# laboshinl/loam_velodyne

Hardware: AMD Instinct MI355X
Metric: sweeps/sec (64-ring, 1M-pt map): feature extraction + odometry + scan-to-map registration (higher is better)
Workload: dtype f32

## Files before the change

### loam_velodyne_amd/csrc/odometry.hip

```cpp
#include "odometry.hpp"
#include "odom_schedule.hpp"
#include "pinned_copy.hpp"
#include <chrono>
#include <cstring>
#include <type_traits>

namespace loamx {

constexpr int OD_THREADS = 256;
constexpr int OD_TR_STRIDE = OD_THREADS + 2;
constexpr int OD_PART_STRIDE = 2 * (2 * 16 * LX_NSUM) + 16;
[[maybe_unused]] constexpr int OD_PART_TS = 2 * (2 * 16 * LX_NSUM);

__device__ inline void sincos_f(float a, float& s, float& c) { sincosf(a, &s, &c); }

__device__ inline void transform_to_start(const float* T, float scan_period, const float4 pi, float& x, float& y, float& z) {
  const float s = (1.f / scan_period) * (pi.w - (float)(int)pi.w);
  x = pi.x - s * T[3];
  y = pi.y - s * T[4];
  z = pi.z - s * T[5];
  float sx, cx, sy, cy, sz, cz;
  sincos_f(-s * T[0], sx, cx);
  sincos_f(-s * T[1], sy, cy);
  sincos_f(-s * T[2], sz, cz);
// ... 107 lines not shown
      v = cell_start[((uint32_t)z * g.ny + y) * g.nx + xx];
    }
  }
  uint32_t acc = 0;
#pragma unroll
  for (int r = 0; r < 9; r++) {
    const uint32_t b = (uint32_t)__shfl((int)v, 2 * r, 64), e = (uint32_t)__shfl((int)v, 2 * r + 1, 64);
    B.O[r] = b - acc;
    acc += e > b ? e - b : 0u;
    B.E[r] = acc;
  }
  B.total = acc;
}
#ifndef OD_BLK_CACHE
#define OD_BLK_CACHE 2
#endif
struct Block27First { float4 p[OD_BLK_CACHE > 0 ? OD_BLK_CACHE : 1]; };
template <bool LOAD_FIRST, class F>
__device__ inline void block27_scan(const Block27& B, const float4* __restrict__ sorted, int lane, Block27First& first, F&& visit) {
  for (uint32_t c0 = (uint32_t)lane; c0 < B.total; c0 += 4 * 64) {
    const bool first_trip = c0 == (uint32_t)lane;
    uint32_t pos[4];
    float4 p[4];
#pragma unroll
    for (int u = 0; u < 4; u++) {
      const uint32_t cc = c0 + 64u * u;
      uint32_t o = B.O[8];
#pragma unroll
      for (int k = 7; k >= 0; k--) o = cc < B.E[k] ? B.O[k] : o;
      pos[u] = cc < B.total ? cc + o : B.O[0];
    }
    if (LOAD_FIRST || !first_trip) {
#pragma unroll
      for (int u = 0; u < 4; u++) p[u] = sorted[pos[u]];
      if (LOAD_FIRST && first_trip) {
#pragma unroll
        for (int u = 0; u < OD_BLK_CACHE; u++) first.p[u] = p[u];
      }
    } else {
#pragma unroll
      for (int u = OD_BLK_CACHE; u < 4; u++) p[u] = sorted[pos[u]];
#pragma unroll
      for (int u = 0; u < OD_BLK_CACHE; u++) p[u] = first.p[u];
    }
#pragma unroll
    for (int u = 0; u < 4; u++) visit(p[u], (c0 + 64u * u) < B.total);
  }
}
__device__ inline int nn1_block(const GridDesc& g, const Block27& B, const float4* __restrict__ sorted, const uint32_t* __restrict__ cell_start,
                                float qx, float qy, float qz, int lane, uint32_t& w_out, Block27First& first) {
  float lbest = 25.0f;
  uint32_t lw = 0xffffffffu;
  block27_scan<true>(B, sorted, lane, first, [&](const float4& p, bool valid) {
    const float dx = qx - p.x, dy2 = qy - p.y, dz2 = qz - p.z;
    const float d2 = dx * dx + dy2 * dy2 + dz2 * dz2;
    const uint32_t w = __float_as_uint(p.w);
    if (valid && (d2 < lbest || (d2 == lbest && lw != 0xffffffffu && (w & OD_IDX_MASK) < (lw & OD_IDX_MASK)))) { lbest = d2; lw = w; }
  });
  float d = lbest;
  int j = lw == 0xffffffffu ? -1 : (int)(lw & OD_IDX_MASK), o_ = lw == 0xffffffffu ? 0x7fffffff : (int)(lw & OD_IDX_MASK);
  int ring = (int)(lw >> 24);
  {
#pragma unroll
    for (int off = 32; off > 0; off >>= 1) {
      const float od = __shfl_xor(d, off, 64);
      const int oj = __shfl_xor(j, off, 64), oo = __shfl_xor(o_, off, 64), orr = __shfl_xor(ring, off, 64);
      if (od < d || (od == d && oo < o_)) { d = od; j = oj; o_ = oo; ring = orr; }
    }
  }
  const float h = 1.0f / g.inv_h;
  if (j >= 0 && d < 25.0f && d <= h * h) { w_out = ((uint32_t)ring << 24) | (uint32_t)j; return j; }
  const int id = nn1_shells(g, sorted, cell_start, qx, qy, qz, lane, 2, (j >= 0 && d < 25.0f) ? d : 25.0f, (j >= 0 && d < 25.0f) ? j : -1);
  w_out = id == j ? (((uint32_t)ring << 24) | (uint32_t)j) : (0xff000000u | (uint32_t)(id < 0 ? 0 : id));
  return id;
}

constexpr int OD_RF_N = 320;
#ifdef LOAMX_PROF_CORR
__device__ unsigned long long g_corr_ts[3][16];
#define OC_TS(k) do { if (blockIdx.y == 0 && lane == 0 && ts_slot >= 0) g_corr_ts[ts_slot][k] = wall_clock64(); } while (0)
#else
#define OC_TS(k) do { } while (0)
#endif
__global__ __launch_bounds__(256) OD_CORR_ATTR void k_odom_corr_grid(OdomProblem* __restrict__ probs, OdomParams P, uint32_t* __restrict__ patch_dst, uint4 patch) {
  if (patch_dst && blockIdx.x == 0 && blockIdx.y == 0 && threadIdx.x == 0) { patch_dst[0] = patch.x; patch_dst[1] = patch.y; patch_dst[2] = patch.z; }
  OdomProblem& pb = probs[blockIdx.y];
  if (pb.done) return;
  const int lane = threadIdx.x & 63, wid = threadIdx.x >> 6;
  const int nSharp = (int)pb.n_sharp, nFlat = (int)pb.n_flat;
  int f;
  {
    const int x = (int)(blockIdx.x % 8), j = (int)(blockIdx.x / 8);
    const int sS = (int)((long long)x * nSharp / 8), nS = (int)((long long)(x + 1) * nSharp / 8) - sS;
    const int sF = (int)((long long)x * nFlat / 8), nF = (int)((long long)(x + 1) * nFlat / 8) - sF;
    const int fl = 4 * j + wid;
    if (fl >= nS + nF) return;
    f = fl < nS ? sS + fl : nSharp + sF + (fl - nS);
  }
#ifdef LOAMX_PROF_CORR
  const int ts_slot = f == nSharp / 2 ? 0 : f == nSharp + nFlat / 2 ? 1 : f == nSharp + nFlat - 1 ? 2 : -1;
#endif
  OC_TS(0);
  float T[6];
#pragma unroll
  for (int k = 0; k < 6; k++) T[k] = pb.transform[k];
  const bool corner = f < nSharp;
  const float4 pi = corner ? pb.sharp[f] : pb.flat[f - nSharp];
  const uint32_t* __restrict__ tbl = corner ? pb.rf_corner : pb.rf_surf;
  const int e0 = max((int)pi.w - 8, 0);
  uint32_t tv = 0u, unordered_epoch = 0u;
  if (tbl) {
    if (e0 + lane < OD_RF_N - 1) tv = tbl[e0 + lane];
    unordered_epoch = tbl[OD_RF_N - 1];
  }
  float x, y, z;
  transform_to_start(T, P.scan_period, pi, x, y, z);
  const GridDescB gd = corner ? *pb.lc_desc : *pb.ls_desc;
  const float4* __restrict__ sorted = pb.sorted;
  const uint32_t* __restrict__ cell_start = pb.cell_table + gd.cell_base;
  OC_TS(1);
  Block27 B;
  block27_build(gd.g, cell_start, x, y, z, lane, B);
  OC_TS(2);
  uint32_t wbest = 0u;
  Block27First first;
  const int closest = nn1_block(gd.g, B, sorted, cell_start, x, y, z, lane, wbest, first);
  OC_TS(3);
  if (closest < 0) {
    if (lane == 0) { pb.ind[5 * f] = -1; pb.ind[5 * f + 1] = -1; pb.ind[5 * f + 2] = -1; }
    return;
  }
  const float4* last = corner ? pb.last_corner : pb.last_surf;
  const int nLast = corner ? (int)pb.n_last_corner : (int)pb.n_last_surf;
  const int nCur = corner ? nSharp : nFlat;
  const int bound = nCur < nLast ? nCur : nLast;
  const int cscan = (wbest >> 24) != 255u ? (int)(wbest >> 24) : (int)last[closest].w;
  float d2 = 25.f, d3 = 25.f;
  int j2 = -1, j3 = -1, o2 = 0x7fffffff, o3 = 0x7fffffff;
  auto better = [](float d, int order, float dbest, int obest) { return d < dbest || (d == dbest && obest != 0x7fffffff && order < obest); };

  bool via_block = false;
  if (tbl && unordered_epoch != pb.rf_epoch && cscan < 255 && B.total > 0u) {
    const unsigned long long valid = __ballot(e0 + lane < OD_RF_N - 1 && (tv >> 24) == pb.rf_epoch);
    auto first_from = [&](int ring) -> int {
      const int k = ring - e0;
      if (k >= 64) return nLast;
      const unsigned long long m = k <= 0 ? valid : (valid >> k) << k;
      if (!m) return nLast;
      const int w = (int)((uint32_t)__shfl((int)tv, __builtin_ctzll(m), 64) & OD_IDX_MASK);
      return w < nLast ? w : nLast;
    };
    if (cscan - 2 >= e0 || e0 == 0) {
      const int wlo = min(first_from(cscan - 2), closest);
      const int whi = closest + 1 < bound ? max(min(bound, first_from(cscan + 3)), closest + 1) : closest + 1;
      const unsigned walk = (unsigned)(closest - wlo) + (unsigned)(whi - (closest + 1));
      via_block = walk > B.total + 128u;
    }
  }
  OC_TS(4);
  if (via_block) {
    block27_scan<false>(B, sorted, lane, first, [&](const float4& p, bool ok) {
      const uint32_t w = __float_as_uint(p.w);
      const int j = (int)(w & OD_IDX_MASK), ring = (int)(w >> 24);
      const float d = sqd(p, x, y, z);
      if (ok && j > closest && j < bound && ring <= cscan + 2) {
        const int order = j - (closest + 1);
        if (corner) {
          if (ring > cscan && better(d, order, d2, o2)) { d2 = d; j2 = j; o2 = order; }
        } else {
          if (ring <= cscan) { if (better(d, order, d2, o2)) { d2 = d; j2 = j; o2 = order; } }
          else { if (better(d, order, d3, o3)) { d3 = d; j3 = j; o3 = order; } }
        }
      } else if (ok && j < closest && ring >= cscan - 2) {
        const int order = 0x40000000 + (closest - 1 - j);
        if (corner) {
          if (ring < cscan && better(d, order, d2, o2)) { d2 = d; j2 = j; o2 = order; }
        } else {
          if (ring >= cscan) { if (better(d, order, d2, o2)) { d2 = d; j2 = j; o2 = order; } }
          else { if (better(d, order, d3, o3)) { d3 = d; j3 = j; o3 = order; } }
        }
      }
    });
    wave_argmin(d2, j2, o2);
    if (!corner) wave_argmin(d3, j3, o3);
    const float h = 1.0f / gd.g.inv_h, h2 = h * h;
    via_block = d2 < h2 && (corner || d3 < h2);
    if (!via_block) { d2 = d3 = 25.f; j2 = j3 = -1; o2 = o3 = 0x7fffffff; }
  }
  OC_TS(5);
  if (!via_block) {
    int baseF = closest + 1, baseB = closest - 1;
    bool stopF = baseF >= bound, stopB = baseB < 0;
    while (!stopF || !stopB) {
      float4 qf[4], qb[4];
      if (!stopF) {
#pragma unroll
        for (int u = 0; u < 4; u++) {
          const int j = baseF + 64 * u + lane;
          qf[u] = j < bound ? last[j] : make_float4(0.f, 0.f, 0.f, 0.f);
        }
      }
      if (!stopB) {
#pragma unroll
        for (int u = 0; u < 4; u++) {
          const int j = baseB - 64 * u - lane;
          qb[u] = j >= 0 ? last[j] : make_float4(0.f, 0.f, 0.f, 0.f);
        }
      }
      if (!stopF) {
        bool stop = false;
#pragma unroll
        for (int u = 0; u < 4; u++) {
          if (stop) continue;
          const int j = baseF + 64 * u + lane;
          const bool in = j < bound;
          const int ring = (int)qf[u].w;
          const bool brk = in && ((double)ring > (double)cscan + 2.5);
          const unsigned long long mb = __ballot(brk);
          const int fb = mb ? __builtin_ctzll(mb) : 64;
          if (in && lane < fb) {
            const float d = sqd(qf[u], x, y, z);
            const int order = j - (closest + 1);
            if (corner) {
              if (ring > cscan && better(d, order, d2, o2)) { d2 = d; j2 = j; o2 = order; }
            } else {
              if (ring <= cscan) { if (better(d, order, d2, o2)) { d2 = d; j2 = j; o2 = order; } }
              else { if (better(d, order, d3, o3)) { d3 = d; j3 = j; o3 = order; } }
            }
          }
          if (mb) stop = true;
        }
        baseF += 256;
        stopF = stop || baseF >= bound;
      }
      if (!stopB) {
        bool stop = false;
#pragma unroll
        for (int u = 0; u < 4; u++) {
          if (stop) continue;
          const int j = baseB - 64 * u - lane;
          const bool in = j >= 0;
          const int ring = (int)qb[u].w;
          const bool brk = in && ((double)ring < (double)cscan - 2.5);
          const unsigned long long mb = __ballot(brk);
          const int fb = mb ? __builtin_ctzll(mb) : 64;
          if (in && lane < fb) {
            const float d = sqd(qb[u], x, y, z);
            const int order = 0x40000000 + (closest - 1 - j);
            if (corner) {
              if (ring < cscan && better(d, order, d2, o2)) { d2 = d; j2 = j; o2 = order; }
            } else {
              if (ring >= cscan) { if (better(d, order, d2, o2)) { d2 = d; j2 = j; o2 = order; } }
              else { if (better(d, order, d3, o3)) { d3 = d; j3 = j; o3 = order; } }
            }
          }
          if (mb) stop = true;
        }
        baseB -= 256;
        stopB = stop || baseB < 0;
      }
    }
    wave_argmin(d2, j2, o2);
    if (!corner) wave_argmin(d3, j3, o3);
  }
  OC_TS(6);
  if (lane == 0) {
    pb.ind[5 * f] = closest;
    pb.ind[5 * f + 1] = j2;
    pb.ind[5 * f + 2] = corner ? -1 : j3;
  }
#ifdef LOAMX_PROF_CORR
  if (blockIdx.y == 0 && lane == 0 && ts_slot >= 0) {
    g_corr_ts[ts_slot][7] = wall_clock64();
    g_corr_ts[ts_slot][8] = (unsigned long long)B.total; g_corr_ts[ts_slot][9] = (unsigned long long)via_block;
    g_corr_ts[ts_slot][10] = (unsigned long long)closest; g_corr_ts[ts_slot][11] = (unsigned long long)cscan;
  }
#endif
}

#ifdef LOAMX_PROF_LM
#define LM_TS(k) do { if (blockIdx.x == 0 && blockIdx.y == 0 && tid == 0 && iter == it_begin + 1) pb.part[OD_PART_TS + (k)] = (double)wall_clock64(); } while (0)
#else
#define LM_TS(k) do { } while (0)
#endif
#ifndef OD_LM_WAVES
#define OD_LM_WAVES 3
#endif
#ifndef OD_LM_WAVES_MIN
#define OD_LM_WAVES_MIN 3
#endif
#define OD_LM_ATTR __attribute__((amdgpu_waves_per_eu(OD_LM_WAVES_MIN, OD_LM_WAVES)))
#pragma clang diagnostic push
#pragma clang diagnostic ignored "-Wpass-failed"
template <int OD_FPT>
__global__ __launch_bounds__(OD_THREADS) OD_LM_ATTR void k_odom_lm(OdomProblem* __restrict__ probs, OdomParams P, int iter0, int n_iters) {
  OdomProblem& pb = probs[blockIdx.y];
  if (pb.done) return;
  const unsigned NB = gridDim.x;
  const int tid = threadIdx.x;
  const int nSharp = (int)pb.n_sharp, nFlat = (int)pb.n_flat, nFeat = nSharp + nFlat;
  __shared__ float T[6];
  __shared__ float trig[6];
  __shared__ double red[8][LX_NSUM];
  using TrT = typename std::conditional<OD_FPT == 1, float, double>::type;
  __shared__ TrT tr[LX_NSUM * OD_TR_STRIDE];
  __shared__ int sh_done, sh_degen, sh_abort;
  __shared__ float matP[36];
  __shared__ float ws[216];
  __shared__ double parts[16 * LX_NSUM];
  __shared__ float AtA[36], AtB[6];
  if (tid < 6) {
    T[tid] = pb.transform[tid];
    const double ang = (double)pb.transform[tid >> 1];
    trig[tid] = (float)((tid & 1) ? cos(ang) : sin(ang));
  }
  const unsigned xtag = pb.xchg_epoch << 8;
  if (tid == 0) { sh_done = 0; sh_abort = 0; sh_degen = pb.stats.degenerate; }
  if (tid < 36) matP[tid] = pb.matP[tid];
  __syncthreads();

  float4 fpo[OD_FPT], ft1[OD_FPT], ft2[OD_FPT], ft3[OD_FPT];
  bool fvalid[OD_FPT], fcorner[OD_FPT];
#pragma unroll
  for (int u = 0; u < OD_FPT; u++) {
    const int f = (u * (int)NB + (int)blockIdx.x) * OD_THREADS + tid;
    fvalid[u] = false;
    fcorner[u] = f < nSharp;
    fpo[u] = ft1[u] = ft2[u] = ft3[u] = make_float4(0.f, 0.f, 0.f, 0.f);
    if (f < nFeat) {
      const int i1 = pb.ind[5 * f], i2 = pb.ind[5 * f + 1], i3 = pb.ind[5 * f + 2];
      if (fcorner[u] ? (i2 >= 0) : (i2 >= 0 && i3 >= 0)) {
        fvalid[u] = true;
        fpo[u] = fcorner[u] ? pb.sharp[f] : pb.flat[f - nSharp];
        const float4* last = fcorner[u] ? pb.last_corner : pb.last_surf;
        ft1[u] = last[i1];
        ft2[u] = last[i2];
        if (!fcorner[u]) ft3[u] = last[i3];
      }
    }
  }

  const int it_begin = iter0, it_end = iter0 + n_iters;
  for (int iter = it_begin; iter < it_end; iter++) {
    LM_TS(0);
    LM_TS(1);
    double v[OD_FPT == 1 ? 1 : LX_NSUM];
    float a1[6] = {0.f, 0.f, 0.f, 0.f, 0.f, 0.f}, bb1 = 0.f;
    bool sel1 = false;
#pragma unroll
    for (int k = 0; k < (OD_FPT == 1 ? 1 : LX_NSUM); k++) v[k] = 0.0;
#pragma unroll
    for (int u = 0; u < OD_FPT; u++) {
      if (!fvalid[u]) continue;
      const bool corner = fcorner[u];
      const float4 po = fpo[u];
      float cx = 0.f, cy = 0.f, cz = 0.f, ci = 0.f;
      bool sel = false;
      {
        float x0, y0, z0;
        transform_to_start(T, P.scan_period, po, x0, y0, z0);
        if (corner) {
// ... 361 lines not shown
void OdometryBatch::lt_resolve_() {
  for (auto& c : lt_) {
    if (!c.pending || !c.pairs) continue;
    if (hipEventQuery(c.ev[3 * (c.pairs - 1) + 2]) != hipSuccess) { (void)hipGetLastError(); continue; }
    for (int k = 0; k < c.pairs; k++) {
      float a = 0.f, b = 0.f;
      if (hipEventElapsedTime(&a, c.ev[3 * k], c.ev[3 * k + 1]) != hipSuccess || hipEventElapsedTime(&b, c.ev[3 * k + 1], c.ev[3 * k + 2]) != hipSuccess) { (void)hipGetLastError(); continue; }
      if (c.iters[k] > 0) {
        lt_tot_.corr_ms += a; lt_tot_.corr_launches++; lt_tot_.corr_features += c.feats[k];
        lt_tot_.lm_ms += b; lt_tot_.lm_launches++; lt_tot_.lm_iterations += (uint64_t)c.iters[k]; lt_tot_.lm_bytes += c.bytes[k];
      } else {
        lt_tot_.corr_noop_ms += a; lt_tot_.corr_noop_launches++;
        lt_tot_.lm_noop_ms += b; lt_tot_.lm_noop_launches++;
      }
    }
    c.pending = false;
  }
}
OdometryBatch::LaunchTotals OdometryBatch::launch_totals() {
  std::lock_guard<std::mutex> lk(lt_mu_);
  lt_resolve_();
  return lt_tot_;
}

void odom_set_imu(OdomStream& S, const float* t);
ToEndParams odom_to_end_params(const OdomStream& S, float scan_period, bool enabled);
void odom_integrate_pose(OdomStream& S);

void OdometryBatch::update_imu(uint32_t s, const float* t) { odom_set_imu(*streams_[s], t); }

ToEndParams OdometryBatch::to_end_params(uint32_t s, bool enabled) const { return odom_to_end_params(*streams_[s], params.scan_period, enabled); }

void OdometryBatch::to_end_device(uint32_t s, float4* pts, uint32_t n) {
  if (!n) return;
  hipLaunchKernelGGL(k_transform_to_end, dim3((n + 255) / 256), dim3(256), 0, st_, pts, n, to_end_params(s, true));
}

void odom_integrate_pose(OdomStream& S) {
  HAngle rx, ry, rz;
  accumulate_rotation(S.transform_sum.rot_x, S.transform_sum.rot_y, S.transform_sum.rot_z, -S.transform.rot_x,
                      HAngle((float)(-S.transform.rot_y.r * 1.05)), -S.transform.rot_z, rx, ry, rz);
  HVec3 v{S.transform.pos.x - S.imu_shift.x, S.transform.pos.y - S.imu_shift.y, (float)(S.transform.pos.z * 1.05 - S.imu_shift.z)};
  h_rot_zxy(v, rz, rx, ry);
  HVec3 trans{S.transform_sum.pos.x - v.x, S.transform_sum.pos.y - v.y, S.transform_sum.pos.z - v.z};
  plugin_imu_rotation(rx, ry, rz, S.imu_pitch_start, S.imu_yaw_start, S.imu_roll_start, S.imu_pitch_end, S.imu_yaw_end,
                      S.imu_roll_end, rx, ry, rz);
  S.transform_sum.rot_x = rx; S.transform_sum.rot_y = ry; S.transform_sum.rot_z = rz;
  S.transform_sum.pos = trans;
}
void odom_set_imu(OdomStream& S, const float* t) {
  S.imu_pitch_start = HAngle(t[0]); S.imu_yaw_start = HAngle(t[1]); S.imu_roll_start = HAngle(t[2]);
  S.imu_pitch_end = HAngle(t[3]); S.imu_yaw_end = HAngle(t[4]); S.imu_roll_end = HAngle(t[5]);
  S.imu_shift = {t[6], t[7], t[8]};
  S.imu_velo = {t[9], t[10], t[11]};
}
ToEndParams odom_to_end_params(const OdomStream& S, float scan_period, bool enabled) {
  ToEndParams P;
  S.transform.get(P.T);
  const HAngle* ta[3] = {&S.transform.rot_x, &S.transform.rot_y, &S.transform.rot_z};
  const HAngle* sa[3] = {&S.imu_pitch_start, &S.imu_yaw_start, &S.imu_roll_start};
  const HAngle* ea[3] = {&S.imu_pitch_end, &S.imu_yaw_end, &S.imu_roll_end};
  for (int k = 0; k < 3; k++) {
    P.sT[k] = ta[k]->s; P.cT[k] = ta[k]->c;
    P.s_start[k] = sa[k]->s; P.c_start[k] = sa[k]->c;
    P.s_end[k] = ea[k]->s; P.c_end[k] = ea[k]->c;
  }
  P.shift[0] = S.imu_shift.x; P.shift[1] = S.imu_shift.y; P.shift[2] = S.imu_shift.z;
  P.scan_period = scan_period;
  P.enabled = enabled ? 1 : 0;
  return P;
}

struct OdometryBatch::Pass {
  const OdomInput* in;
  int* rc;
  uint32_t ns, K;
  std::vector<OdomInput> in_late;
  bool late_pending = false, patch_pending = false;
  uint32_t n_corner_all = 0, n_all = 0;
  const float4 *src_c = nullptr, *src_s = nullptr;
  std::vector<uint32_t> active;
  uint32_t max_feat = 0, max_sharp = 0, max_flat = 0;
  LtCall* lt = nullptr;
};

void OdometryBatch::process(const OdomInput* in, int* rc, bool defer_tail) {
  TraceRange trace_range("loamx:odometry");
  LX_HIP(hipSetDevice(device_));
  if (up_pending_) {
    LX_HIP(hipEventSynchronize(ev_up_));
    up_pending_ = false;
  }
  Pass p{in, rc, n_streams(), 2 * n_streams()};
  stage_clouds_(p);
  build_problems_(p);
  upload_(p);
  launch_pairs_(p);
  enqueue_tail_(p);
  if (!p.active.empty()) collect_(p);
  integrate_poses_(p);
  if (!defer_tail) {
    LX_HIP(hipStreamSynchronize(st_));
    tail_pending_ = false;
  }
}

void OdometryBatch::stage_clouds_(Pass& p) {
  const uint32_t ns = p.ns;
  p.late_pending = ns == 1 && (bool)late_less_flat;
  if (p.late_pending) {
    p.in_late.assign(p.in, p.in + ns);
    p.in_late[0].less_flat = nullptr; p.in_late[0].n_less_flat = 0;
    p.in = p.in_late.data();
  }
  const OdomInput* in = p.in;
  for (uint32_t s = 0; s < ns; s++) {
    h_cur_off_[s + 1] = h_cur_off_[s] + in[s].n_less_sharp;
    if (s > 0) LX_REQUIRE(in[s].less_sharp == in[s - 1].less_sharp + in[s - 1].n_less_sharp || in[s].n_less_sharp == 0 || in[s - 1].n_less_sharp == 0,
                          "less_sharp clouds of the streams must be contiguous");
  }
  for (uint32_t s = 0; s < ns; s++) h_cur_off_[ns + s + 1] = h_cur_off_[ns + s] + in[s].n_less_flat;
  const uint32_t n_corner_all = p.n_corner_all = h_cur_off_[ns], n_all = p.n_all = h_cur_off_[p.K];
  cur_.reserve((size_t)n_all + (p.late_pending ? late_bound : 0u) + 1);
  bool contig_c = true, contig_s = true;
  for (uint32_t s = 1; s < ns; s++) {
    contig_c = contig_c && in[s].less_sharp == in[s - 1].less_sharp + in[s - 1].n_less_sharp;
    contig_s = contig_s && in[s].less_flat == in[s - 1].less_flat + in[s - 1].n_less_flat;
  }
  if (contig_c && contig_s) { p.src_c = in[0].less_sharp; p.src_s = in[0].less_flat; return; }
  if (contig_c) {
    if (n_corner_all) LX_HIP(hipMemcpyAsync(cur_.p, in[0].less_sharp, sizeof(float4) * n_corner_all, hipMemcpyDeviceToDevice, st_));
  } else {
    for (uint32_t s = 0; s < ns; s++)
      if (in[s].n_less_sharp) LX_HIP(hipMemcpyAsync(cur_.p + h_cur_off_[s], in[s].less_sharp, sizeof(float4) * in[s].n_less_sharp, hipMemcpyDeviceToDevice, st_));
  }
  if (contig_s) {
    if (n_all > n_corner_all) LX_HIP(hipMemcpyAsync(cur_.p + n_corner_all, in[0].less_flat, sizeof(float4) * (n_all - n_corner_all), hipMemcpyDeviceToDevice, st_));
  } else {
    for (uint32_t s = 0; s < ns; s++)
      if (in[s].n_less_flat) LX_HIP(hipMemcpyAsync(cur_.p + h_cur_off_[ns + s], in[s].less_flat, sizeof(float4) * in[s].n_less_flat, hipMemcpyDeviceToDevice, st_));
  }
}

void OdometryBatch::resolve_late_(Pass& p) {
  if (!p.late_pending) return;
  p.late_pending = false;
  const float4* pts = nullptr;
  uint32_t n = 0;
  late_less_flat(pts, n);
  LX_REQUIRE(n <= late_bound, "internal: the late less-flat cloud is larger than its announced bound");
  p.in_late[0].less_flat = pts; p.in_late[0].n_less_flat = n;
  h_cur_off_[p.ns + 1] = h_cur_off_[p.ns] + n;
  p.n_all = h_cur_off_[p.K];
  p.src_s = pts;
  p.patch_pending = true;
}
void OdometryBatch::flush_patch_(Pass& p) {
  if (!p.patch_pending) return;
  p.patch_pending = false;
  h_off_late_.reserve(p.K + 1);
  memcpy(h_off_late_.p, h_cur_off_.data(), sizeof(uint32_t) * (p.K + 1));
  LX_HIP(hipMemcpyAsync(d_cur_off_.p, h_off_late_.p, sizeof(uint32_t) * (p.K + 1), hipMemcpyHostToDevice, st_));
  LX_HIP(hipEventRecord(ev_up_, st_));
}

void OdometryBatch::build_problems_(Pass& p) {
  const uint32_t ns = p.ns;
  xchg_epoch_ = xchg_epoch_ % 0xffffffu + 1u;
  std::vector<uint32_t> ind_off(ns + 1, 0);
  for (uint32_t s = 0; s < ns; s++) ind_off[s + 1] = ind_off[s] + 5 * (p.in[s].n_sharp + p.in[s].n_flat) + 5;
  ind_.reserve(ind_off[ns] + 8);
  for (uint32_t s = 0; s < ns; s++) {
    OdomStream& S = *streams_[s];
    const OdomInput& I = p.in[s];
    if (!S.inited) {
      S.transform_sum.rot_x = HAngle(S.transform_sum.rot_x.r + S.imu_pitch_start.r);
      S.transform_sum.rot_z = HAngle(S.transform_sum.rot_z.r + S.imu_roll_start.r);
      p.rc[s] = LOAMX_SKIPPED;
      continue;
    }
    p.rc[s] = LOAMX_OK;
    S.frame++;
    S.transform.pos.x -= S.imu_velo.x * params.scan_period;
    S.transform.pos.y -= S.imu_velo.y * params.scan_period;
    S.transform.pos.z -= S.imu_velo.z * params.scan_period;
    S.stats = {0, 0, (int)S.frame, 0};
    if (S.n_last_corner > 10 && S.n_last_surf > 100) {
      OdomProblem& pb = h_prob_.p[p.active.size()];
      pb.sharp = I.sharp; pb.n_sharp = I.n_sharp;
      pb.flat = I.flat; pb.n_flat = I.n_flat;
      pb.last_corner = last_.p + h_last_off_[s]; pb.n_last_corner = S.n_last_corner;
      pb.last_surf = last_.p + h_last_off_[ns + s]; pb.n_last_surf = S.n_last_surf;
      pb.sorted = index_.sorted();
      pb.cell_table = index_.cell_table();
      pb.lc_desc = index_.desc(s);
      pb.ls_desc = index_.desc(ns + s);
      pb.ind = ind_.p + ind_off[s];
      S.transform.get(pb.transform);
      pb.stats = {0, 0, 0, 0};
      pb.done = 0;
      pb.ticket = 0;
      pb.xchg_epoch = xchg_epoch_;
      pb.stream_id = (int)s;
      pb.host_mirror = h_mirror_.p + p.active.size();
      pb.te_out = te_.p + s;
      pb.part = part_.p + (size_t)p.active.size() * OD_PART_STRIDE;
      pb.err_word = h_err_.p;
      pb.rf_corner = rf_.p + (size_t)s * OD_RF_N;
      pb.rf_surf = rf_.p + (size_t)(ns + s) * OD_RF_N;
      pb.rf_epoch = rf_epoch_;
      p.max_feat = std::max(p.max_feat, I.n_sharp + I.n_flat);
      p.max_sharp = std::max(p.max_sharp, I.n_sharp);
      p.max_flat = std::max(p.max_flat, I.n_flat);
      p.active.push_back(s);
    }
  }
  if (p.max_feat > 32 * OD_THREADS) throw Error(LOAMX_E_CAPACITY, "more than 8192 sharp+flat features in one sweep");
}

void OdometryBatch::upload_(Pass& p) {
  for (uint32_t s = 0; s < p.ns; s++) h_te_.p[s] = to_end_params(s, p.rc[s] == LOAMX_OK);
  memcpy(h_off_pin_.p, h_cur_off_.data(), sizeof(uint32_t) * (p.K + 1));
  LX_HIP(hipMemcpyAsync(up_dev_.p, up_host_.p, up_bytes_, hipMemcpyHostToDevice, st_));
  index_.prepare(p.K);
  if (!ev_up_) LX_HIP(hipEventCreateWithFlags(&ev_up_, hipEventDisableTiming));
  LX_HIP(hipEventRecord(ev_up_, st_));
  up_pending_ = true;
}

static dim3 odom_corr_grid(uint32_t max_sharp, uint32_t max_flat, uint32_t na) {
  return dim3(8 * (((max_sharp + 7) / 8 + (max_flat + 7) / 8 + 3) / 4), na);
}
OdometryBatch::LmGeometry OdometryBatch::lm_geometry_(uint32_t max_feat) {
#ifdef OD_LM_HALF_WGS
  const uint32_t nb = std::min<uint32_t>(16u, std::max<uint32_t>(1u, (max_feat + 2 * OD_THREADS - 1) / (2 * OD_THREADS)));
#else
  const uint32_t nb = std::min<uint32_t>(16u, (max_feat + OD_THREADS - 1) / OD_THREADS);
#endif
  const bool two = max_feat > nb * OD_THREADS;
  if (!lm_slots_[two]) {
    int per_cu = 0;
    if (two) LX_HIP(hipOccupancyMaxActiveBlocksPerMultiprocessor(&per_cu, k_odom_lm<2>, OD_THREADS, 0));
    else LX_HIP(hipOccupancyMaxActiveBlocksPerMultiprocessor(&per_cu, k_odom_lm<1>, OD_THREADS, 0));
    hipDeviceProp_t prop;
    LX_HIP(hipGetDeviceProperties(&prop, device_));
    lm_slots_[two] = (uint32_t)std::max(per_cu, 1) * (uint32_t)std::max(prop.multiProcessorCount, 1);
  }
  return {nb, two, std::max<uint32_t>(1u, (lm_slots_[two] / 2) / nb)};
}

void OdometryBatch::enqueue_corr_(Pass& p, int k) {
  LtCall* lt = p.lt;
  const int lk = lt && k < LT_MAXP ? k : -1;
  if (lk >= 0) {
    for (int e = 0; e < 3; e++) if (!lt->ev[3 * lk + e]) LX_HIP(hipEventCreate(&lt->ev[3 * lk + e]));
    LX_HIP(hipEventRecord(lt->ev[3 * lk], st_));
  }
  uint32_t* pd = nullptr;
  uint4 pv = make_uint4(0u, 0u, 0u, 0u);
  if (p.patch_pending) { p.patch_pending = false; pd = d_cur_off_.p; pv = make_uint4(h_cur_off_[0], h_cur_off_[1], h_cur_off_[2], 0u); }
  hipLaunchKernelGGL(k_odom_corr_grid, odom_corr_grid(p.max_sharp, p.max_flat, (uint32_t)p.active.size()), dim3(256), 0, st_, prob_.p, params, pd, pv);
  if (lk >= 0) LX_HIP(hipEventRecord(lt->ev[3 * lk + 1], st_));
}
void OdometryBatch::enqueue_lm_(Pass& p, int k) {
  LtCall* lt = p.lt;
  const uint32_t na = (uint32_t)p.active.size();
  const int it0 = 5 * k;
  const int nit = std::min(5, params.max_iterations - it0);
  const int lk = lt && k < LT_MAXP ? k : -1;
  const LmGeometry g = lm_geometry_(p.max_feat);
  for (uint32_t a0 = 0; a0 < na; a0 += g.chunk) {
    const uint32_t nc = std::min(g.chunk, na - a0);
    if (g.two) hipLaunchKernelGGL(k_odom_lm<2>, dim3(g.nb, nc), dim3(OD_THREADS), 0, st_, prob_.p + a0, params, it0, nit);
    else hipLaunchKernelGGL(k_odom_lm<1>, dim3(g.nb, nc), dim3(OD_THREADS), 0, st_, prob_.p + a0, params, it0, nit);
  }
  if (lk >= 0) { LX_HIP(hipEventRecord(lt->ev[3 * lk + 2], st_)); lt->pairs = lk + 1; }
}

struct OdometryBatch::PairOps {
  OdometryBatch& o; Pass& p;
  void corr(int k) { o.enqueue_corr_(p, k); }
  void lm(int k) { o.enqueue_lm_(p, k); }
  void after_first() { o.resolve_late_(p); }
  bool behind(int want) const {
    const volatile OdomProblem* hm = o.h_mirror_.p;
    for (size_t a = 0; a < p.active.size(); a++) if (hm[a].done == 0 && hm[a].stats.iterations < want) return true;
    return false;
  }
  bool converged() const { return !behind(o.params.max_iterations); }
  bool wait_settled(int k) const {
    const int want = std::min(5 * (k + 1), o.params.max_iterations);
    const auto t_in = std::chrono::steady_clock::now();
    for (unsigned spins = 0; behind(want);) {
      if ((++spins & 255u) == 0u && std::chrono::steady_clock::now() - t_in > std::chrono::milliseconds(20)) return false;
      cpu_relax();
    }
    return true;
  }
};

void OdometryBatch::launch_pairs_(Pass& p) {
  const uint32_t na = (uint32_t)p.active.size();
  if (launch_timing_.load(std::memory_order_relaxed) && na && p.max_feat) {
    std::lock_guard<std::mutex> lk(lt_mu_);
    lt_resolve_();
    LtCall& c = lt_[lt_next_ % LT_RING];
    if (!c.pending) { p.lt = &c; lt_next_++; c.pairs = 0; }
  }
  if (!na) return;
  if (p.max_feat) {
    const char* e = getenv("LOAMX_ODOM_PAIRS");
    const OdomPairMode mode = !e ? OdomPairMode::Lag : !strcmp(e, "all") ? OdomPairMode::All : !strcmp(e, "exact") ? OdomPairMode::Exact : !strcmp(e, "lag2") ? OdomPairMode::Lag2 : OdomPairMode::Lag;
    for (uint32_t a = 0; a < na; a++) { h_mirror_.p[a].done = 0; h_mirror_.p[a].stats.iterations = 0; }
    odom_schedule_pairs(PairOps{*this, p}, mode, (params.max_iterations + 4) / 5, pred_pairs_);
  }
  if (!p.max_feat) LX_HIP(hipMemcpyAsync(h_mirror_.p, prob_.p, sizeof(OdomProblem) * na, hipMemcpyDeviceToHost, st_));
  if (!ev_pose_) LX_HIP(hipEventCreateWithFlags(&ev_pose_, hipEventDisableTiming));
  LX_HIP(hipEventRecord(ev_pose_, st_));
  if (!p.max_feat) hipLaunchKernelGGL(k_te_patch, dim3((na + 63) / 64), dim3(64), 0, st_, prob_.p, na, te_.p);
}

void OdometryBatch::enqueue_tail_(Pass& p) {
  static const bool fuse_bounds = !(diag_env("LOAMX_BB_FUSED") && atoi(diag_env("LOAMX_BB_FUSED")) == 0);
  resolve_late_(p);
  flush_patch_(p);
  if (p.n_all) {
    if (++rf_epoch_ > 255u) rf_epoch_ = 1u;
    hipLaunchKernelGGL(k_transform_to_end_batch, dim3((p.n_all + 255) / 256), dim3(256), 0, st_, cur_.p, p.n_all, d_cur_off_.p, p.K, p.ns, te_.p, p.src_c,
                       p.src_s, p.n_corner_all, fuse_bounds ? index_.d_bounds() : nullptr, rf_.p, rf_epoch_);
  }
  {
    float4* q = cur_.p; size_t c = cur_.cap;
    DevBuf<float4>& oldest = older_[keep_ - 2];
    cur_.p = oldest.p; cur_.cap = oldest.cap;
    for (int k = keep_ - 2; k > 0; k--) { older_[k].p = older_[k - 1].p; older_[k].cap = older_[k - 1].cap; }
    older_[0].p = last_.p; older_[0].cap = last_.cap;
    last_.p = q; last_.cap = c;
  }
  h_last_off_ = h_cur_off_;
// ... 196 lines not shown
```

Before: 16150.

## Pass odometry problem head through kernel arguments instead of a host-to-device upload

Adds a variant of the correspondence kernel that receives per-stream problem descriptors, to-end params and offsets as a large kernel-argument struct. Block 0 of each stream then writes these into device problem structs. This skips the separate hipMemcpyAsync upload and its event when the stream count fits, removing one transfer from the per-pass chain. The risks are a bigger argument segment and possible ordering hazards, because other blocks read pb fields that block 0 writes in the same launch.

```diff
diff --git a/loam_velodyne_amd/csrc/odom_corr_kernel.inc b/loam_velodyne_amd/csrc/odom_corr_kernel.inc
--- /dev/null
+++ b/loam_velodyne_amd/csrc/odom_corr_kernel.inc
@@ -0,0 +1,201 @@
+#if OC_VARIANT == 0
+__global__ __launch_bounds__(256) OD_CORR_ATTR void OC_KERNEL(OdomProblem* __restrict__ probs, OdomParams P, uint32_t* __restrict__ patch_dst, uint4 patch) {
+  if (patch_dst && blockIdx.x == 0 && blockIdx.y == 0 && threadIdx.x == 0) { patch_dst[0] = patch.x; patch_dst[1] = patch.y; patch_dst[2] = patch.z; }
+  OdomProblem& pb = probs[blockIdx.y];
+  if (pb.done) return;
+#else
+__global__ __launch_bounds__(256) OD_CORR_ATTR void OC_KERNEL(const OdomHeadArgs H, OdomParams P) {
+  odom_head_publish(H);
+  const OdomHeadStream& pb = H.s[blockIdx.y];
+#endif
+  const int lane = threadIdx.x & 63, wid = threadIdx.x >> 6;
+  const int nSharp = (int)pb.n_sharp, nFlat = (int)pb.n_flat;
+  int f;
+  {
+    const int x = (int)(blockIdx.x % 8), j = (int)(blockIdx.x / 8);
+    const int sS = (int)((long long)x * nSharp / 8), nS = (int)((long long)(x + 1) * nSharp / 8) - sS;
+    const int sF = (int)((long long)x * nFlat / 8), nF = (int)((long long)(x + 1) * nFlat / 8) - sF;
+    const int fl = 4 * j + wid;
+    if (fl >= nS + nF) return;
+    f = fl < nS ? sS + fl : nSharp + sF + (fl - nS);
+  }
+#ifdef LOAMX_PROF_CORR
+  const int ts_slot = f == nSharp / 2 ? 0 : f == nSharp + nFlat / 2 ? 1 : f == nSharp + nFlat - 1 ? 2 : -1;
+#endif
+  OC_TS(0);
+  float T[6];
+#pragma unroll
+  for (int k = 0; k < 6; k++) T[k] = pb.transform[k];
+  const bool corner = f < nSharp;
+  const float4 pi = corner ? pb.sharp[f] : pb.flat[f - nSharp];
+  const uint32_t* __restrict__ tbl = corner ? pb.rf_corner : pb.rf_surf;
+  const int e0 = max((int)pi.w - 8, 0);
+  uint32_t tv = 0u, unordered_epoch = 0u;
+  if (tbl) {
+    if (e0 + lane < OD_RF_N - 1) tv = tbl[e0 + lane];
+    unordered_epoch = tbl[OD_RF_N - 1];
+  }
+  float x, y, z;
+  transform_to_start(T, P.scan_period, pi, x, y, z);
+  const GridDescB gd = corner ? *pb.lc_desc : *pb.ls_desc;
+  const float4* __restrict__ sorted = pb.sorted;
+  const uint32_t* __restrict__ cell_start = pb.cell_table + gd.cell_base;
+  OC_TS(1);
+  Block27 B;
+  block27_build(gd.g, cell_start, x, y, z, lane, B);
+  OC_TS(2);
+  uint32_t wbest = 0u;
+  Block27First first;
+  const int closest = nn1_block(gd.g, B, sorted, cell_start, x, y, z, lane, wbest, first);
+  OC_TS(3);
+  if (closest < 0) {
+    if (lane == 0) { pb.ind[5 * f] = -1; pb.ind[5 * f + 1] = -1; pb.ind[5 * f + 2] = -1; }
+    return;
+  }
+  const float4* last = corner ? pb.last_corner : pb.last_surf;
+  const int nLast = corner ? (int)pb.n_last_corner : (int)pb.n_last_surf;
+  const int nCur = corner ? nSharp : nFlat;
+  const int bound = nCur < nLast ? nCur : nLast;
+  const int cscan = (wbest >> 24) != 255u ? (int)(wbest >> 24) : (int)last[closest].w;
+  float d2 = 25.f, d3 = 25.f;
+  int j2 = -1, j3 = -1, o2 = 0x7fffffff, o3 = 0x7fffffff;
+  auto better = [](float d, int order, float dbest, int obest) { return d < dbest || (d == dbest && obest != 0x7fffffff && order < obest); };
+
+  bool via_block = false;
+  if (tbl && unordered_epoch != pb.rf_epoch && cscan < 255 && B.total > 0u) {
+    const unsigned long long valid = __ballot(e0 + lane < OD_RF_N - 1 && (tv >> 24) == pb.rf_epoch);
+    auto first_from = [&](int ring) -> int {
+      const int k = ring - e0;
+      if (k >= 64) return nLast;
+      const unsigned long long m = k <= 0 ? valid : (valid >> k) << k;
+      if (!m) return nLast;
+      const int w = (int)((uint32_t)__shfl((int)tv, __builtin_ctzll(m), 64) & OD_IDX_MASK);
+      return w < nLast ? w : nLast;
+    };
+    if (cscan - 2 >= e0 || e0 == 0) {
+      const int wlo = min(first_from(cscan - 2), closest);
+      const int whi = closest + 1 < bound ? max(min(bound, first_from(cscan + 3)), closest + 1) : closest + 1;
+      const unsigned walk = (unsigned)(closest - wlo) + (unsigned)(whi - (closest + 1));
+      via_block = walk > B.total + 128u;
+    }
+  }
+  OC_TS(4);
+  if (via_block) {
+    block27_scan<false>(B, sorted, lane, first, [&](const float4& p, bool ok) {
+      const uint32_t w = __float_as_uint(p.w);
+      const int j = (int)(w & OD_IDX_MASK), ring = (int)(w >> 24);
+      const float d = sqd(p, x, y, z);
+      if (ok && j > closest && j < bound && ring <= cscan + 2) {
+        const int order = j - (closest + 1);
+        if (corner) {
+          if (ring > cscan && better(d, order, d2, o2)) { d2 = d; j2 = j; o2 = order; }
+        } else {
+          if (ring <= cscan) { if (better(d, order, d2, o2)) { d2 = d; j2 = j; o2 = order; } }
+          else { if (better(d, order, d3, o3)) { d3 = d; j3 = j; o3 = order; } }
+        }
+      } else if (ok && j < closest && ring >= cscan - 2) {
+        const int order = 0x40000000 + (closest - 1 - j);
+        if (corner) {
+          if (ring < cscan && better(d, order, d2, o2)) { d2 = d; j2 = j; o2 = order; }
+        } else {
+          if (ring >= cscan) { if (better(d, order, d2, o2)) { d2 = d; j2 = j; o2 = order; } }
+          else { if (better(d, order, d3, o3)) { d3 = d; j3 = j; o3 = order; } }
+        }
+      }
+    });
+    wave_argmin(d2, j2, o2);
+    if (!corner) wave_argmin(d3, j3, o3);
+    const float h = 1.0f / gd.g.inv_h, h2 = h * h;
+    via_block = d2 < h2 && (corner || d3 < h2);
+    if (!via_block) { d2 = d3 = 25.f; j2 = j3 = -1; o2 = o3 = 0x7fffffff; }
+  }
+  OC_TS(5);
+  if (!via_block) {
+    int baseF = closest + 1, baseB = closest - 1;
+    bool stopF = baseF >= bound, stopB = baseB < 0;
+    while (!stopF || !stopB) {
+      float4 qf[4], qb[4];
+      if (!stopF) {
+#pragma unroll
+        for (int u = 0; u < 4; u++) {
+          const int j = baseF + 64 * u + lane;
+          qf[u] = j < bound ? last[j] : make_float4(0.f, 0.f, 0.f, 0.f);
+        }
+      }
+      if (!stopB) {
+#pragma unroll
+        for (int u = 0; u < 4; u++) {
+          const int j = baseB - 64 * u - lane;
+          qb[u] = j >= 0 ? last[j] : make_float4(0.f, 0.f, 0.f, 0.f);
+        }
+      }
+      if (!stopF) {
+        bool stop = false;
+#pragma unroll
+        for (int u = 0; u < 4; u++) {
+          if (stop) continue;
+          const int j = baseF + 64 * u + lane;
+          const bool in = j < bound;
+          const int ring = (int)qf[u].w;
+          const bool brk = in && ((double)ring > (double)cscan + 2.5);
+          const unsigned long long mb = __ballot(brk);
+          const int fb = mb ? __builtin_ctzll(mb) : 64;
+          if (in && lane < fb) {
+            const float d = sqd(qf[u], x, y, z);
+            const int order = j - (closest + 1);
+            if (corner) {
+              if (ring > cscan && better(d, order, d2, o2)) { d2 = d; j2 = j; o2 = order; }
+            } else {
+              if (ring <= cscan) { if (better(d, order, d2, o2)) { d2 = d; j2 = j; o2 = order; } }
+              else { if (better(d, order, d3, o3)) { d3 = d; j3 = j; o3 = order; } }
+            }
+          }
+          if (mb) stop = true;
+        }
+        baseF += 256;
+        stopF = stop || baseF >= bound;
+      }
+      if (!stopB) {
+        bool stop = false;
+#pragma unroll
+        for (int u = 0; u < 4; u++) {
+          if (stop) continue;
+          const int j = baseB - 64 * u - lane;
+          const bool in = j >= 0;
+          const int ring = (int)qb[u].w;
+          const bool brk = in && ((double)ring < (double)cscan - 2.5);
+          const unsigned long long mb = __ballot(brk);
+          const int fb = mb ? __builtin_ctzll(mb) : 64;
+          if (in && lane < fb) {
+            const float d = sqd(qb[u], x, y, z);
+            const int order = 0x40000000 + (closest - 1 - j);
+            if (corner) {
+              if (ring < cscan && better(d, order, d2, o2)) { d2 = d; j2 = j; o2 = order; }
+            } else {
+              if (ring >= cscan) { if (better(d, order, d2, o2)) { d2 = d; j2 = j; o2 = order; } }
+              else { if (better(d, order, d3, o3)) { d3 = d; j3 = j; o3 = order; } }
+            }
+          }
+          if (mb) stop = true;
+        }
+        baseB -= 256;
+        stopB = stop || baseB < 0;
+      }
+    }
+    wave_argmin(d2, j2, o2);
+    if (!corner) wave_argmin(d3, j3, o3);
+  }
+  OC_TS(6);
+  if (lane == 0) {
+    pb.ind[5 * f] = closest;
+    pb.ind[5 * f + 1] = j2;
+    pb.ind[5 * f + 2] = corner ? -1 : j3;
+  }
+#ifdef LOAMX_PROF_CORR
+  if (blockIdx.y == 0 && lane == 0 && ts_slot >= 0) {
+    g_corr_ts[ts_slot][7] = wall_clock64();
+    g_corr_ts[ts_slot][8] = (unsigned long long)B.total; g_corr_ts[ts_slot][9] = (unsigned long long)via_block;
+    g_corr_ts[ts_slot][10] = (unsigned long long)closest; g_corr_ts[ts_slot][11] = (unsigned long long)cscan;
+  }
+#endif
+}
diff --git a/loam_velodyne_amd/csrc/odometry.hip b/loam_velodyne_amd/csrc/odometry.hip
--- a/loam_velodyne_amd/csrc/odometry.hip
+++ b/loam_velodyne_amd/csrc/odometry.hip
@@ -213,201 +213,82 @@
 #else
 #define OC_TS(k) do { } while (0)
 #endif
-__global__ __launch_bounds__(256) OD_CORR_ATTR void k_odom_corr_grid(OdomProblem* __restrict__ probs, OdomParams P, uint32_t* __restrict__ patch_dst, uint4 patch) {
-  if (patch_dst && blockIdx.x == 0 && blockIdx.y == 0 && threadIdx.x == 0) { patch_dst[0] = patch.x; patch_dst[1] = patch.y; patch_dst[2] = patch.z; }
-  OdomProblem& pb = probs[blockIdx.y];
-  if (pb.done) return;
-  const int lane = threadIdx.x & 63, wid = threadIdx.x >> 6;
-  const int nSharp = (int)pb.n_sharp, nFlat = (int)pb.n_flat;
-  int f;
-  {
-    const int x = (int)(blockIdx.x % 8), j = (int)(blockIdx.x / 8);
-    const int sS = (int)((long long)x * nSharp / 8), nS = (int)((long long)(x + 1) * nSharp / 8) - sS;
-    const int sF = (int)((long long)x * nFlat / 8), nF = (int)((long long)(x + 1) * nFlat / 8) - sF;
-    const int fl = 4 * j + wid;
-    if (fl >= nS + nF) return;
-    f = fl < nS ? sS + fl : nSharp + sF + (fl - nS);
-  }
-#ifdef LOAMX_PROF_CORR
-  const int ts_slot = f == nSharp / 2 ? 0 : f == nSharp + nFlat / 2 ? 1 : f == nSharp + nFlat - 1 ? 2 : -1;
-#endif
-  OC_TS(0);
-  float T[6];
-#pragma unroll
-  for (int k = 0; k < 6; k++) T[k] = pb.transform[k];
-  const bool corner = f < nSharp;
-  const float4 pi = corner ? pb.sharp[f] : pb.flat[f - nSharp];
-  const uint32_t* __restrict__ tbl = corner ? pb.rf_corner : pb.rf_surf;
-  const int e0 = max((int)pi.w - 8, 0);
-  uint32_t tv = 0u, unordered_epoch = 0u;
-  if (tbl) {
-    if (e0 + lane < OD_RF_N - 1) tv = tbl[e0 + lane];
-    unordered_epoch = tbl[OD_RF_N - 1];
-  }
-  float x, y, z;
-  transform_to_start(T, P.scan_period, pi, x, y, z);
-  const GridDescB gd = corner ? *pb.lc_desc : *pb.ls_desc;
-  const float4* __restrict__ sorted = pb.sorted;
-  const uint32_t* __restrict__ cell_start = pb.cell_table + gd.cell_base;
-  OC_TS(1);
-  Block27 B;
-  block27_build(gd.g, cell_start, x, y, z, lane, B);
-  OC_TS(2);
-  uint32_t wbest = 0u;
-  Block27First first;
-  const int closest = nn1_block(gd.g, B, sorted, cell_start, x, y, z, lane, wbest, first);
-  OC_TS(3);
-  if (closest < 0) {
-    if (lane == 0) { pb.ind[5 * f] = -1; pb.ind[5 * f + 1] = -1; pb.ind[5 * f + 2] = -1; }
-    return;
-  }
-  const float4* last = corner ? pb.last_corner : pb.last_surf;
-  const int nLast = corner ? (int)pb.n_last_corner : (int)pb.n_last_surf;
-  const int nCur = corner ? nSharp : nFlat;
-  const int bound = nCur < nLast ? nCur : nLast;
-  const int cscan = (wbest >> 24) != 255u ? (int)(wbest >> 24) : (int)last[closest].w;
-  float d2 = 25.f, d3 = 25.f;
-  int j2 = -1, j3 = -1, o2 = 0x7fffffff, o3 = 0x7fffffff;
-  auto better = [](float d, int order, float dbest, int obest) { return d < dbest || (d == dbest && obest != 0x7fffffff && order < obest); };
-
-  bool via_block = false;
-  if (tbl && unordered_epoch != pb.rf_epoch && cscan < 255 && B.total > 0u) {
-    const unsigned long long valid = __ballot(e0 + lane < OD_RF_N - 1 && (tv >> 24) == pb.rf_epoch);
-    auto first_from = [&](int ring) -> int {
-      const int k = ring - e0;
-      if (k >= 64) return nLast;
-      const unsigned long long m = k <= 0 ? valid : (valid >> k) << k;
-      if (!m) return nLast;
-      const int w = (int)((uint32_t)__shfl((int)tv, __builtin_ctzll(m), 64) & OD_IDX_MASK);
-      return w < nLast ? w : nLast;
-    };
-    if (cscan - 2 >= e0 || e0 == 0) {
-      const int wlo = min(first_from(cscan - 2), closest);
-      const int whi = closest + 1 < bound ? max(min(bound, first_from(cscan + 3)), closest + 1) : closest + 1;
-      const unsigned walk = (unsigned)(closest - wlo) + (unsigned)(whi - (closest + 1));
-      via_block = walk > B.total + 128u;
-    }
-  }
-  OC_TS(4);
-  if (via_block) {
-    block27_scan<false>(B, sorted, lane, first, [&](const float4& p, bool ok) {
-      const uint32_t w = __float_as_uint(p.w);
-      const int j = (int)(w & OD_IDX_MASK), ring = (int)(w >> 24);
-      const float d = sqd(p, x, y, z);
-      if (ok && j > closest && j < bound && ring <= cscan + 2) {
-        const int order = j - (closest + 1);
-        if (corner) {
-          if (ring > cscan && better(d, order, d2, o2)) { d2 = d; j2 = j; o2 = order; }
-        } else {
-          if (ring <= cscan) { if (better(d, order, d2, o2)) { d2 = d; j2 = j; o2 = order; } }
-          else { if (better(d, order, d3, o3)) { d3 = d; j3 = j; o3 = order; } }
-        }
-      } else if (ok && j < closest && ring >= cscan - 2) {
-        const int order = 0x40000000 + (closest - 1 - j);
-        if (corner) {
-          if (ring < cscan && better(d, order, d2, o2)) { d2 = d; j2 = j; o2 = order; }
-        } else {
-          if (ring >= cscan) { if (better(d, order, d2, o2)) { d2 = d; j2 = j; o2 = order; } }
-          else { if (better(d, order, d3, o3)) { d3 = d; j3 = j; o3 = order; } }
-        }
-      }
-    });
-    wave_argmin(d2, j2, o2);
-    if (!corner) wave_argmin(d3, j3, o3);
-    const float h = 1.0f / gd.g.inv_h, h2 = h * h;
-    via_block = d2 < h2 && (corner || d3 < h2);
-    if (!via_block) { d2 = d3 = 25.f; j2 = j3 = -1; o2 = o3 = 0x7fffffff; }
-  }
-  OC_TS(5);
-  if (!via_block) {
-    int baseF = closest + 1, baseB = closest - 1;
-    bool stopF = baseF >= bound, stopB = baseB < 0;
-    while (!stopF || !stopB) {
-      float4 qf[4], qb[4];
-      if (!stopF) {
-#pragma unroll
-        for (int u = 0; u < 4; u++) {
-          const int j = baseF + 64 * u + lane;
-          qf[u] = j < bound ? last[j] : make_float4(0.f, 0.f, 0.f, 0.f);
-        }
-      }
-      if (!stopB) {
-#pragma unroll
-        for (int u = 0; u < 4; u++) {
-          const int j = baseB - 64 * u - lane;
-          qb[u] = j >= 0 ? last[j] : make_float4(0.f, 0.f, 0.f, 0.f);
-        }
-      }
-      if (!stopF) {
-        bool stop = false;
-#pragma unroll
-        for (int u = 0; u < 4; u++) {
-          if (stop) continue;
-          const int j = baseF + 64 * u + lane;
-          const bool in = j < bound;
-          const int ring = (int)qf[u].w;
-          const bool brk = in && ((double)ring > (double)cscan + 2.5);
-          const unsigned long long mb = __ballot(brk);
-          const int fb = mb ? __builtin_ctzll(mb) : 64;
-          if (in && lane < fb) {
-            const float d = sqd(qf[u], x, y, z);
-            const int order = j - (closest + 1);
-            if (corner) {
-              if (ring > cscan && better(d, order, d2, o2)) { d2 = d; j2 = j; o2 = order; }
-            } else {
-              if (ring <= cscan) { if (better(d, order, d2, o2)) { d2 = d; j2 = j; o2 = order; } }
-              else { if (better(d, order, d3, o3)) { d3 = d; j3 = j; o3 = order; } }
-            }
-          }
-          if (mb) stop = true;
-        }
-        baseF += 256;
-        stopF = stop || baseF >= bound;
-      }
-      if (!stopB) {
-        bool stop = false;
-#pragma unroll
-        for (int u = 0; u < 4; u++) {
-          if (stop) continue;
-          const int j = baseB - 64 * u - lane;
-          const bool in = j >= 0;
-          const int ring = (int)qb[u].w;
-          const bool brk = in && ((double)ring < (double)cscan - 2.5);
-          const unsigned long long mb = __ballot(brk);
-          const int fb = mb ? __builtin_ctzll(mb) : 64;
-          if (in && lane < fb) {
-            const float d = sqd(qb[u], x, y, z);
-            const int order = 0x40000000 + (closest - 1 - j);
-            if (corner) {
-              if (ring < cscan && better(d, order, d2, o2)) { d2 = d; j2 = j; o2 = order; }
-            } else {
-              if (ring >= cscan) { if (better(d, order, d2, o2)) { d2 = d; j2 = j; o2 = order; } }
-              else { if (better(d, order, d3, o3)) { d3 = d; j3 = j; o3 = order; } }
-            }
-          }
-          if (mb) stop = true;
-        }
-        baseB -= 256;
-        stopB = stop || baseB < 0;
-      }
-    }
-    wave_argmin(d2, j2, o2);
-    if (!corner) wave_argmin(d3, j3, o3);
-  }
-  OC_TS(6);
-  if (lane == 0) {
-    pb.ind[5 * f] = closest;
-    pb.ind[5 * f + 1] = j2;
-    pb.ind[5 * f + 2] = corner ? -1 : j3;
-  }
-#ifdef LOAMX_PROF_CORR
-  if (blockIdx.y == 0 && lane == 0 && ts_slot >= 0) {
-    g_corr_ts[ts_slot][7] = wall_clock64();
-    g_corr_ts[ts_slot][8] = (unsigned long long)B.total; g_corr_ts[ts_slot][9] = (unsigned long long)via_block;
-    g_corr_ts[ts_slot][10] = (unsigned long long)closest; g_corr_ts[ts_slot][11] = (unsigned long long)cscan;
-  }
-#endif
-}
+constexpr uint32_t OD_ARG_STREAMS = 8;
+struct OdomHeadStream {
+  const float4 *sharp, *flat, *last_corner, *last_surf, *sorted;
+  const uint32_t* cell_table;
+  const GridDescB *lc_desc, *ls_desc;
+  int* ind;
+  ToEndParams* te_out;
+  OdomProblem* host_mirror;
+  double* part;
+  const uint32_t *rf_corner, *rf_surf;
+  uint32_t* err_word;
+  uint32_t n_sharp, n_flat, n_last_corner, n_last_surf;
+  float transform[6];
+  int stream_id;
+  uint32_t xchg_epoch, rf_epoch;
+};
+struct OdomHeadArgs {
+  OdomHeadStream s[OD_ARG_STREAMS];
+  ToEndParams te[OD_ARG_STREAMS];
+  uint32_t off[2 * OD_ARG_STREAMS + 1];
+  uint32_t ns;
+  OdomProblem* probs;
+  ToEndParams* te_dst;
+  uint32_t* off_dst;
+};
+static_assert(sizeof(OdomHeadArgs) <= 3072, "the pass's head has to fit the kernel-argument segment beside the other arguments");
+__device__ inline void odom_head_publish(const OdomHeadArgs& H) {
+  if (blockIdx.x != 0) return;
+  const int tid = (int)threadIdx.x;
+  const OdomHeadStream& hs = H.s[blockIdx.y];
+  OdomProblem& pb = H.probs[blockIdx.y];
+  if (tid < 36) pb.matP[tid] = 0.f;
+  if (tid >= 64 && tid < 70) pb.transform[tid - 64] = hs.transform[tid - 64];
+  if (tid == 128) {
+    pb.sharp = hs.sharp; pb.n_sharp = hs.n_sharp;
+    pb.flat = hs.flat; pb.n_flat = hs.n_flat;
+    pb.last_corner = hs.last_corner; pb.n_last_corner = hs.n_last_corner;
+    pb.last_surf = hs.last_surf; pb.n_last_surf = hs.n_last_surf;
+    pb.sorted = hs.sorted;
+    pb.cell_table = hs.cell_table;
+    pb.lc_desc = hs.lc_desc;
+    pb.ls_desc = hs.ls_desc;
+    pb.ind = hs.ind;
+  }
+  if (tid == 192) {
+    pb.stats = {0, 0, 0, 0};
+    pb.done = 0;
+    pb.stream_id = hs.stream_id;
+    pb.te_out = hs.te_out;
+    pb.host_mirror = hs.host_mirror;
+    pb.ticket = 0u;
+    pb.xchg_epoch = hs.xchg_epoch;
+    pb.part = hs.part;
+    pb.rf_corner = hs.rf_corner;
+    pb.rf_surf = hs.rf_surf;
+    pb.rf_epoch = hs.rf_epoch;
+    pb.err_word = hs.err_word;
+  }
+  if (blockIdx.y == 0) {
+    static_assert(sizeof(ToEndParams) % 4 == 0, "copied word by word");
+    const uint32_t* src = reinterpret_cast<const uint32_t*>(H.te);
+    uint32_t* dst = reinterpret_cast<uint32_t*>(H.te_dst);
+    for (uint32_t w = (uint32_t)tid; w < H.ns * (uint32_t)(sizeof(ToEndParams) / 4); w += 256u) dst[w] = src[w];
+    for (uint32_t w = (uint32_t)tid; w < 2u * H.ns + 1u; w += 256u) H.off_dst[w] = H.off[w];
+  }
+}
+#define OC_KERNEL k_odom_corr_grid
+#define OC_VARIANT 0
+#include "odom_corr_kernel.inc"
+#undef OC_KERNEL
+#undef OC_VARIANT
+#define OC_KERNEL k_odom_corr_head
+#define OC_VARIANT 1
+#include "odom_corr_kernel.inc"
+#undef OC_KERNEL
+#undef OC_VARIANT
 
 #ifdef LOAMX_PROF_LM
 #define LM_TS(k) do { if (blockIdx.x == 0 && blockIdx.y == 0 && tid == 0 && iter == it_begin + 1) pb.part[OD_PART_TS + (k)] = (double)wall_clock64(); } while (0)
@@ -935,6 +816,7 @@
   std::vector<uint32_t> active;
   uint32_t max_feat = 0, max_sharp = 0, max_flat = 0;
   LtCall* lt = nullptr;
+  bool head_in_args = false;
 };
 
 void OdometryBatch::process(const OdomInput* in, int* rc, bool defer_tail) {
@@ -947,6 +829,10 @@
   Pass p{in, rc, n_streams(), 2 * n_streams()};
   stage_clouds_(p);
   build_problems_(p);
+  {
+    const char* e = getenv("LOAMX_ODOM_CHAIN");
+    p.head_in_args = !(e && !strcmp(e, "plain")) && p.ns <= OD_ARG_STREAMS && !p.late_pending && !p.active.empty() && p.max_feat > 0;
+  }
   upload_(p);
   launch_pairs_(p);
   enqueue_tail_(p);
@@ -1074,6 +960,10 @@
 void OdometryBatch::upload_(Pass& p) {
   for (uint32_t s = 0; s < p.ns; s++) h_te_.p[s] = to_end_params(s, p.rc[s] == LOAMX_OK);
   memcpy(h_off_pin_.p, h_cur_off_.data(), sizeof(uint32_t) * (p.K + 1));
+  if (p.head_in_args) {
+    index_.prepare(p.K);
+    return;
+  }
   LX_HIP(hipMemcpyAsync(up_dev_.p, up_host_.p, up_bytes_, hipMemcpyHostToDevice, st_));
   index_.prepare(p.K);
   if (!ev_up_) LX_HIP(hipEventCreateWithFlags(&ev_up_, hipEventDisableTiming));
@@ -1108,6 +998,26 @@
   if (lk >= 0) {
     for (int e = 0; e < 3; e++) if (!lt->ev[3 * lk + e]) LX_HIP(hipEventCreate(&lt->ev[3 * lk + e]));
     LX_HIP(hipEventRecord(lt->ev[3 * lk], st_));
+  }
+  if (k == 0 && p.head_in_args) {
+    OdomHeadArgs H;
+    memset(&H, 0, sizeof(H));
+    for (size_t a = 0; a < p.active.size(); a++) {
+      const OdomProblem& pb = h_prob_.p[a];
+      OdomHeadStream& hs = H.s[a];
+      hs.sharp = pb.sharp; hs.flat = pb.flat; hs.last_corner = pb.last_corner; hs.last_surf = pb.last_surf; hs.sorted = pb.sorted;
+      hs.cell_table = pb.cell_table; hs.lc_desc = pb.lc_desc; hs.ls_desc = pb.ls_desc; hs.ind = pb.ind; hs.te_out = pb.te_out;
+      hs.host_mirror = pb.host_mirror; hs.part = pb.part; hs.rf_corner = pb.rf_corner; hs.rf_surf = pb.rf_surf; hs.err_word = pb.err_word;
+      hs.n_sharp = pb.n_sharp; hs.n_flat = pb.n_flat; hs.n_last_corner = pb.n_last_corner; hs.n_last_surf = pb.n_last_surf;
+      memcpy(hs.transform, pb.transform, sizeof(hs.transform));
+      hs.stream_id = pb.stream_id; hs.xchg_epoch = pb.xchg_epoch; hs.rf_epoch = pb.rf_epoch;
+    }
+    memcpy(H.te, h_te_.p, sizeof(ToEndParams) * p.ns);
+    memcpy(H.off, h_cur_off_.data(), sizeof(uint32_t) * (p.K + 1));
+    H.ns = p.ns; H.probs = prob_.p; H.te_dst = te_.p; H.off_dst = d_cur_off_.p;
+    hipLaunchKernelGGL(k_odom_corr_head, odom_corr_grid(p.max_sharp, p.max_flat, (uint32_t)p.active.size()), dim3(256), 0, st_, H, params);
+    if (lk >= 0) LX_HIP(hipEventRecord(lt->ev[3 * lk + 1], st_));
+    return;
   }
   uint32_t* pd = nullptr;
   uint4 pv = make_uint4(0u, 0u, 0u, 0u);
```

Result: no change. 16130 (-0.1%).
